# AI4Science-WestlakeU/safediffcon

Measured on AMD Instinct MI355X. Metric: sampled control trajectories/sec (1000-step DDPM), higher is better.
Workload: dtype f32; 1 GPU; C4: 2D smoke Unet3D_with_Conv3D dim=64 (1,2,4) state (B,32,7,64,64), B=64 per GPU, guided 1000-step DDPM, conformal quantile on; batch_per_gpu=64, global_batch=64, step=U-Net + guidance + posterior update of the whole batch, one hipGraph replay, parallelism=batch-sharded x1, no data-path collective, conv_precision=fp32

## Files before the change

### safediffcon_amd/csrc/sdc_conv_stem_x3.hip

```cpp
#include "sdc_conv.h"

using namespace sdcconv;

namespace {

typedef __bf16 bf16x8 __attribute__((ext_vector_type(8)));

constexpr int SX_BM = 64, SX_BN = 256, SX_NT = 256;

struct StemX3Args {
    const float* x;
    const __bf16* wb;
    const float* bias;
    float* y;
    int64_t xs[5], ys[5];
    int B, Cin, Cout, oD, oH, W, lgW;
    int kD;
    int Hs, NR;
    int Ntot, ntiles, mtiles;
    int itemsB;
    int plane;
};

__device__ __forceinline__ void split3(float x, __bf16& h, __bf16& m, __bf16& l) {
#pragma clang fp contract(off)
    h = (__bf16)x;
    const float r = x - (float)h;
    m = (__bf16)r;
    l = (__bf16)(r - (float)m);
}

template <int KH, int ITB>
__global__ __launch_bounds__(SX_NT) __attribute__((amdgpu_waves_per_eu(1))) SDC_NO_DS_MERGE void conv_stem_x3_kernel(const StemX3Args a) {
    constexpr int TAPS = KH * 7;
    constexpr int NS = (TAPS + 1) / 2;
    constexpr int SS = KH == 7 ? 5 : NS;
    constexpr int NSUB = NS / SS;
    static_assert(NSUB * SS == NS, "whole sub-stages");
    constexpr int HH = KH - 1;
    constexpr int APC = SS * SX_BM * 32;
    constexpr int ASZ = 3 * APC;
    constexpr int NIA = 3 * SS * SX_BM * 2;
    constexpr int ITA = (NIA + SX_NT - 1) / SX_NT;
    extern __shared__ __attribute__((aligned(16))) char lds[];

    const int tid = threadIdx.x, lane = tid & 63, wave = tid >> 6;
    const int l31 = lane & 31, lh = lane >> 5;
    const int W = a.W, RP = W + 6;
    const int BIMG = a.NR * RP * 16;
    const int logical = xcd_tile(blockIdx.x, a.ntiles * a.mtiles);
    const int mt = logical % a.mtiles, nt = logical / a.mtiles;
    const int m0 = mt * SX_BM, n0 = nt * SX_BN;
    const int r0 = n0 >> a.lgW;
    const int plane0 = r0 / a.oH, oh0 = r0 - plane0 * a.oH;
    const int GR = a.Hs + HH;

    int64_t bb[ITB];
    int bod[ITB], bdst[ITB];
    bool bok[ITB];
#pragma unroll
    for (int k = 0; k < ITB; ++k) {
        const int it = tid + k * SX_NT;
        const int w = it & (W - 1);
        const int sr = it >> a.lgW;
        int pl, ih;
        if (KH == 1) { const int row = r0 + sr; pl = row / a.oH; ih = row - pl * a.oH; }
        else { const int g = sr / GR, q = sr - g * GR; pl = plane0 + g; ih = (g == 0 ? oh0 : 0) - 3 + q; }
        const bool ok = it < a.itemsB && pl < a.B * a.oD && ih >= 0 && ih < a.oH;
        const int b = ok ? pl / a.oD : 0, od = ok ? pl % a.oD : 0, ihc = ok ? ih : 0;
        bok[k] = ok;
        bod[k] = od;
        bb[k] = (int64_t)b * a.xs[0] + (int64_t)od * a.xs[2] + (int64_t)ihc * a.xs[3] + (int64_t)w;
        bdst[k] = ASZ + (sr * RP + w + 3) * 16;
    }
    int aoff[ITA];
#pragma unroll
    for (int k = 0; k < ITA; ++k) {
        const int it = tid + k * SX_NT;
        const int p = it / (SS * 2 * SX_BM), q = it - p * (SS * 2 * SX_BM);
        const int s = q / (2 * SX_BM), r = q - s * (2 * SX_BM);
        aoff[k] = it < NIA ? p * a.plane + (s * a.Cout + m0) * 16 + r * 8 : 0;
    }

    float bv[ITB][8];
    uint4 av[ITA];
    auto load_a = [&](int kd, int sub) {
        const int wst = (kd * NS + sub * SS) * a.Cout * 16;
#pragma unroll
        for (int k = 0; k < ITA; ++k) {
            uint4 v = make_uint4(0u, 0u, 0u, 0u);
            if (tid + k * SX_NT < NIA) v = *reinterpret_cast<const uint4*>(a.wb + wst + aoff[k]);
            av[k] = v;
        }
    };
    auto load_b = [&](int kd) {
        const int dk = kd - a.kD / 2;
#pragma unroll
        for (int k = 0; k < ITB; ++k) {
            const int sd = bod[k] + dk;
            const bool ok = bok[k] && sd >= 0 && sd < a.oD;
            const float* q = a.x + bb[k] + (int64_t)dk * a.xs[2];
#pragma unroll
            for (int i = 0; i < 8; ++i) { bv[k][i] = (ok && i < a.Cin) ? *q : 0.0f; q += a.xs[1]; }
        }
    };
    auto store_a = [&]() {
#pragma unroll
        for (int k = 0; k < ITA; ++k)
            if (tid + k * SX_NT < NIA) *reinterpret_cast<uint4*>(lds + (tid + k * SX_NT) * 16) = av[k];
    };
    auto store_b = [&]() {
#pragma unroll
        for (int k = 0; k < ITB; ++k) {
            if (tid + k * SX_NT < a.itemsB) {
                bf16x8 h, m, l;
#pragma unroll
                for (int i = 0; i < 8; ++i) { __bf16 ph, pm, pl; split3(bv[k][i], ph, pm, pl); h[i] = ph; m[i] = pm; l[i] = pl; }
                *reinterpret_cast<bf16x8*>(lds + bdst[k]) = h;
                *reinterpret_cast<bf16x8*>(lds + bdst[k] + BIMG) = m;
                *reinterpret_cast<bf16x8*>(lds + bdst[k] + 2 * BIMG) = l;
            }
        }
    };

    for (int e = tid; e < 3 * a.NR * 6; e += SX_NT) {
        const int sr = e / 6, c = e - sr * 6;
        *reinterpret_cast<uint4*>(lds + ASZ + (sr * RP + (c < 3 ? c : W + c)) * 16) = make_uint4(0u, 0u, 0u, 0u);
    }

    int bA[2], bB[2], bC[2];
    constexpr int LAST_OFF = 16 * 6;
#pragma unroll
    for (int j = 0; j < 2; ++j) {
        const int p = wave * 64 + 32 * j + l31;
        const bool pok = n0 + p < a.Ntot;
        const int rl = pok ? p >> a.lgW : 0, col = pok ? p & (W - 1) : 0;
        int slot;
        if (KH == 1) slot = rl;
        else {
            const int row = r0 + rl, pl = row / a.oH, oh = row - pl * a.oH, g = pl - plane0;
            slot = g * GR + oh - (g == 0 ? oh0 : 0);
        }
        const int base = ASZ + (slot * RP + col) * 16;
        bA[j] = base + 16 * lh;
        bB[j] = base + lh * (RP * 16 - 16 * 6);
        bC[j] = lh ? ASZ - (HH * RP * 16 + LAST_OFF) : base;
    }
    const int aoffr = l31 * 32 + 16 * lh;
    const int rowb = RP * 16;

    f32x16 acc[2][2], sm[2][2];
#pragma unroll
    for (int i = 0; i < 2; ++i)
#pragma unroll
        for (int j = 0; j < 2; ++j)
#pragma unroll
            for (int r = 0; r < 16; ++r) {
                acc[i][j][r] = 0.0f;
                sm[i][j][r] = 0.0f;
            }

    load_a(0, 0);
    load_b(0);
    for (int kd = 0; kd < a.kD; ++kd) {
#pragma unroll
        for (int sub = 0; sub < NSUB; ++sub) {
            __syncthreads();
            store_a();
            if (sub == 0) store_b();
            __syncthreads();
            if (sub + 1 < NSUB) load_a(kd, sub + 1);
            else if (kd + 1 < a.kD) { load_a(kd + 1, 0); load_b(kd + 1); }
#pragma unroll
            for (int sl = 0; sl < SS; ++sl) {
                const int s = sub * SS + sl;
                const int t0 = 2 * s, kh = t0 / 7, kw = t0 - 7 * kh;
                const int tb = kh * rowb + kw * 16;
                bf16x8 af[2][3], bf[2][3];
#pragma unroll
                for (int i = 0; i < 2; ++i)
#pragma unroll
                    for (int p = 0; p < 3; ++p)
                        af[i][p] = *reinterpret_cast<const bf16x8*>(lds + p * APC + (sl * SX_BM + 32 * i) * 32 + aoffr);
#pragma unroll
                for (int j = 0; j < 2; ++j) {
                    const int bs = (s == NS - 1) ? bC[j] : (kw == 6 ? bB[j] : bA[j]);
#pragma unroll
                    for (int p = 0; p < 3; ++p) bf[j][p] = *reinterpret_cast<const bf16x8*>(lds + bs + tb + p * BIMG);
                }
                constexpr int PA[6] = {2, 1, 0, 1, 0, 0}, PB[6] = {0, 1, 2, 0, 1, 0};
#pragma unroll
                for (int t = 0; t < 6; ++t)
#pragma unroll
                    for (int i = 0; i < 2; ++i)
#pragma unroll
                        for (int j = 0; j < 2; ++j) {
                            f32x16& c = t < 5 ? sm[i][j] : acc[i][j];
                            c = __builtin_amdgcn_mfma_f32_32x32x16_bf16(af[i][PA[t]], bf[j][PB[t]], c, 0, 0, 0);
                        }
            }
        }
    }

#pragma unroll
    for (int i = 0; i < 2; ++i)
#pragma unroll
        for (int j = 0; j < 2; ++j) acc[i][j] += sm[i][j];
    float bz[2][16];
#pragma unroll
    for (int i = 0; i < 2; ++i)
#pragma unroll
        for (int rr = 0; rr < 16; ++rr) bz[i][rr] = 0.0f;
    if (a.bias) {
#pragma unroll
        for (int i = 0; i < 2; ++i)
#pragma unroll
            for (int rr = 0; rr < 16; ++rr) bz[i][rr] = a.bias[m0 + 32 * i + 4 * lh + (rr & 3) + 8 * (rr >> 2)];
    }
#pragma unroll
    for (int j = 0; j < 2; ++j) {
        const int p = n0 + wave * 64 + 32 * j + l31;
        if (p >= a.Ntot) continue;
        const int row = p >> a.lgW, col = p & (W - 1);
        const int pl = row / a.oH, oh = row - pl * a.oH;
        const int b = pl / a.oD, od = pl - b * a.oD;
        float* yp = a.y + (int64_t)b * a.ys[0] + (int64_t)od * a.ys[2] + (int64_t)oh * a.ys[3] + (int64_t)col
                    + (int64_t)(m0 + 4 * lh) * a.ys[1];
#pragma unroll
        for (int i = 0; i < 2; ++i) {
#pragma unroll
            for (int rr = 0; rr < 16; ++rr)
                yp[(int64_t)(32 * i + (rr & 3) + 8 * (rr >> 2)) * a.ys[1]] = acc[i][j][rr] + bz[i][rr];
        }
    }
}

__global__ __launch_bounds__(256) void pack_stem_x3_kernel(const float* __restrict__ w, __bf16* __restrict__ out, int Cout, int Cin, int kD,
                                                           int taps, int NS, int64_t n) {
    const int64_t e = (int64_t)blockIdx.x * 256 + threadIdx.x;
    if (e >= n) return;
    const int ci = (int)(e & 7), h = (int)((e >> 3) & 1);
    int64_t r = e >> 4;
    const int co = (int)(r % Cout); r /= Cout;
    const int s = (int)(r % NS);
    const int kd = (int)(r / NS);
    const int t = 2 * s + h;
    const float v = (ci < Cin && t < taps) ? w[(((int64_t)co * Cin + ci) * kD + kd) * taps + t] : 0.0f;
    __bf16 ph, pm, pl;
    split3(v, ph, pm, pl);
    out[e] = ph; out[n + e] = pm; out[2 * n + e] = pl;
}

}

namespace sdcconv {

int launch_stem_x3(const SdcConvDesc& d, const float* x, const __bf16* wb, const float* bias, float* y, hipStream_t s) {
    SDC_REQUIRE(reinterpret_cast<uintptr_t>(wb) % 16 == 0, SDC_EALIGN, "sdc_conv_stem_x3: the packed weight buffer must be 16-byte aligned");
    const StemShape sh = stem_shape(d);
    const int NS = (d.kH * 7 + 1) / 2, SS = d.kH == 7 ? 5 : NS;
    const size_t lds = (size_t)3 * SS * SX_BM * 32 + (size_t)3 * sh.NR * (d.oW + 6) * 16;
    SDC_REQUIRE(sh.itemsB <= 8 * SX_NT && lds <= 160u * 1024u, SDC_EINVAL, "sdc_conv_stem_x3: staging of %d positions / %zu bytes of LDS",
                sh.itemsB, lds);
    StemX3Args a;
    a.x = x; a.wb = wb; a.bias = bias; a.y = y;
    for (int i = 0; i < 5; ++i) { a.xs[i] = d.x0s[i]; a.ys[i] = d.ys[i]; }
    a.B = d.B; a.Cin = d.Cin0; a.Cout = d.Cout; a.oD = d.oD; a.oH = d.oH; a.W = d.oW;
    a.lgW = d.oW == 16 ? 4 : d.oW == 32 ? 5 : d.oW == 64 ? 6 : 7;
    a.kD = d.kD;
    a.Hs = sh.Hs; a.NR = sh.NR;
    const int64_t ntot = (int64_t)d.B * d.oD * d.oH * d.oW;
    SDC_REQUIRE(ntot < (1ll << 31), SDC_EINVAL, "sdc_conv_stem_x3: too many output positions");
    const int64_t plane = (int64_t)d.kD * NS * d.Cout * 16;
    SDC_REQUIRE(3 * plane < (1ll << 31), SDC_EINVAL, "sdc_conv_stem_x3: weight too large");
    a.plane = (int)plane;
    a.Ntot = (int)ntot;
    a.ntiles = (a.Ntot + SX_BN - 1) / SX_BN; a.mtiles = d.Cout / SX_BM;
    a.itemsB = sh.itemsB;
    SDC_REQUIRE((int64_t)a.ntiles * a.mtiles < (1ll << 31), SDC_EINVAL, "sdc_conv_stem_x3: grid too large");
    const dim3 grid((unsigned)(a.ntiles * a.mtiles));
#define STEM_LAUNCH(KH, ITB)                                                                                        \
    do {                                                                                                            \
        static std::atomic<uint64_t> attr{0};                                                                       \
        SDC_LDS_OPTIN(attr, (conv_stem_x3_kernel<KH, ITB>), 160 * 1024, "sdc_conv_stem_x3");                        \
        hipLaunchKernelGGL((conv_stem_x3_kernel<KH, ITB>), grid, dim3(SX_NT), lds, s, a);                           \
    } while (0)
    if (d.kH == 1) STEM_LAUNCH(1, 1);
    else if (sh.itemsB <= 2 * SX_NT) STEM_LAUNCH(7, 2);
    else if (sh.itemsB <= 4 * SX_NT) STEM_LAUNCH(7, 4);
    else STEM_LAUNCH(7, 8);
#undef STEM_LAUNCH
    return sdc::check_launch("sdc_conv_stem_x3");
}

}

extern "C" size_t sdc_pack_stem_x3_bytes(int Cout, int Cin, int kD, int kH, int kW) {
    return 3 * sdc_pack_stem_f16_bytes(Cout, Cin, kD, kH, kW);
}

extern "C" int sdc_pack_stem_x3(const float* w, void* out, int Cout, int Cin, int kD, int kH, int kW, void* stream) {
    SDC_REQUIRE(w && out, SDC_ENULL, "sdc_pack_stem_x3: null pointer");
    SDC_REQUIRE(sdc_pack_stem_x3_bytes(Cout, Cin, kD, kH, kW) > 0, SDC_EINVAL,
                "sdc_pack_stem_x3: taps 1x1x7, 1x7x7 or 7x7x7 and 1 <= Cin <= 8 (got %dx%dx%d, Cin %d, Cout %d)", kD, kH, kW, Cin, Cout);
    const int NS = (kH * 7 + 1) / 2;
    const int64_t n = (int64_t)kD * NS * Cout * 16;
    SDC_REQUIRE(n / 256 + 1 < (1ll << 31), SDC_EINVAL, "sdc_pack_stem_x3: weight too large");
    hipLaunchKernelGGL(pack_stem_x3_kernel, dim3((unsigned)((n + 255) / 256)), dim3(256), 0, sdc::as_stream(stream), w,
                       reinterpret_cast<__bf16*>(out), Cout, Cin, kD, kH * 7, NS, n);
    return sdc::check_launch("sdc_pack_stem_x3");
}
```

Measured before the change: 0.2930 trajectories/s.

## Double-buffer weight staging and software-pipeline fragment reads in bf16x3 stem conv

Adds a PIPE variant of the 7x7 bf16x3 stem convolution. It double-buffers the weight tile in LDS and prefetches the next sub-stage's fragments into registers while the current MFMAs run. Scheduling barriers interleave LDS reads with MFMAs, and the number of block-wide syncs per sub-stage drops. This targets exposed LDS and global latency in a single-wave-per-EU kernel, at the cost of more LDS and more registers for the doubled fragments. It also adds debug knobs gated behind an experiments macro.

```diff
diff --git a/safediffcon_amd/csrc/sdc_conv_stem_x3.hip b/safediffcon_amd/csrc/sdc_conv_stem_x3.hip
--- a/safediffcon_amd/csrc/sdc_conv_stem_x3.hip
+++ b/safediffcon_amd/csrc/sdc_conv_stem_x3.hip
@@ -20,6 +20,12 @@
     int Ntot, ntiles, mtiles;
     int itemsB;
     int plane;
+#ifdef SDC_KERNEL_EXPERIMENTS
+    int dbg;
+#define SX_DBG(a) ((a).dbg)
+#else
+#define SX_DBG(a) 0
+#endif
 };
 
 __device__ __forceinline__ void split3(float x, __bf16& h, __bf16& m, __bf16& l) {
@@ -30,7 +36,7 @@
     l = (__bf16)(r - (float)m);
 }
 
-template <int KH, int ITB>
+template <int KH, int ITB, bool PIPE>
 __global__ __launch_bounds__(SX_NT) __attribute__((amdgpu_waves_per_eu(1))) SDC_NO_DS_MERGE void conv_stem_x3_kernel(const StemX3Args a) {
     constexpr int TAPS = KH * 7;
     constexpr int NS = (TAPS + 1) / 2;
@@ -42,6 +48,7 @@
     constexpr int ASZ = 3 * APC;
     constexpr int NIA = 3 * SS * SX_BM * 2;
     constexpr int ITA = (NIA + SX_NT - 1) / SX_NT;
+    constexpr int BOFF = PIPE ? 2 * ASZ : ASZ;
     extern __shared__ __attribute__((aligned(16))) char lds[];
 
     const int tid = threadIdx.x, lane = tid & 63, wave = tid >> 6;
@@ -71,7 +78,7 @@
         bok[k] = ok;
         bod[k] = od;
         bb[k] = (int64_t)b * a.xs[0] + (int64_t)od * a.xs[2] + (int64_t)ihc * a.xs[3] + (int64_t)w;
-        bdst[k] = ASZ + (sr * RP + w + 3) * 16;
+        bdst[k] = BOFF + (sr * RP + w + 3) * 16;
     }
     int aoff[ITA];
 #pragma unroll
@@ -89,7 +96,7 @@
 #pragma unroll
         for (int k = 0; k < ITA; ++k) {
             uint4 v = make_uint4(0u, 0u, 0u, 0u);
-            if (tid + k * SX_NT < NIA) v = *reinterpret_cast<const uint4*>(a.wb + wst + aoff[k]);
+            if (tid + k * SX_NT < NIA && !(SX_DBG(a) & 4)) v = *reinterpret_cast<const uint4*>(a.wb + wst + aoff[k]);
             av[k] = v;
         }
     };
@@ -98,16 +105,16 @@
 #pragma unroll
         for (int k = 0; k < ITB; ++k) {
             const int sd = bod[k] + dk;
-            const bool ok = bok[k] && sd >= 0 && sd < a.oD;
+            const bool ok = bok[k] && sd >= 0 && sd < a.oD && !(SX_DBG(a) & 4);
             const float* q = a.x + bb[k] + (int64_t)dk * a.xs[2];
 #pragma unroll
             for (int i = 0; i < 8; ++i) { bv[k][i] = (ok && i < a.Cin) ? *q : 0.0f; q += a.xs[1]; }
         }
     };
-    auto store_a = [&]() {
+    auto store_a = [&](int abuf) {
 #pragma unroll
         for (int k = 0; k < ITA; ++k)
-            if (tid + k * SX_NT < NIA) *reinterpret_cast<uint4*>(lds + (tid + k * SX_NT) * 16) = av[k];
+            if (tid + k * SX_NT < NIA) *reinterpret_cast<uint4*>(lds + abuf + (tid + k * SX_NT) * 16) = av[k];
     };
     auto store_b = [&]() {
 #pragma unroll
@@ -125,7 +132,7 @@
 
     for (int e = tid; e < 3 * a.NR * 6; e += SX_NT) {
         const int sr = e / 6, c = e - sr * 6;
-        *reinterpret_cast<uint4*>(lds + ASZ + (sr * RP + (c < 3 ? c : W + c)) * 16) = make_uint4(0u, 0u, 0u, 0u);
+        *reinterpret_cast<uint4*>(lds + BOFF + (sr * RP + (c < 3 ? c : W + c)) * 16) = make_uint4(0u, 0u, 0u, 0u);
     }
 
     int bA[2], bB[2], bC[2];
@@ -141,10 +148,10 @@
             const int row = r0 + rl, pl = row / a.oH, oh = row - pl * a.oH, g = pl - plane0;
             slot = g * GR + oh - (g == 0 ? oh0 : 0);
         }
-        const int base = ASZ + (slot * RP + col) * 16;
+        const int base = BOFF + (slot * RP + col) * 16;
         bA[j] = base + 16 * lh;
         bB[j] = base + lh * (RP * 16 - 16 * 6);
-        bC[j] = lh ? ASZ - (HH * RP * 16 + LAST_OFF) : base;
+        bC[j] = lh ? BOFF - (HH * RP * 16 + LAST_OFF) : base;
     }
     const int aoffr = l31 * 32 + 16 * lh;
     const int rowb = RP * 16;
@@ -160,45 +167,114 @@
                 sm[i][j][r] = 0.0f;
             }
 
-    load_a(0, 0);
-    load_b(0);
-    for (int kd = 0; kd < a.kD; ++kd) {
-#pragma unroll
-        for (int sub = 0; sub < NSUB; ++sub) {
-            __syncthreads();
-            store_a();
-            if (sub == 0) store_b();
-            __syncthreads();
-            if (sub + 1 < NSUB) load_a(kd, sub + 1);
-            else if (kd + 1 < a.kD) { load_a(kd + 1, 0); load_b(kd + 1); }
-#pragma unroll
-            for (int sl = 0; sl < SS; ++sl) {
-                const int s = sub * SS + sl;
-                const int t0 = 2 * s, kh = t0 / 7, kw = t0 - 7 * kh;
-                const int tb = kh * rowb + kw * 16;
-                bf16x8 af[2][3], bf[2][3];
-#pragma unroll
-                for (int i = 0; i < 2; ++i)
-#pragma unroll
-                    for (int p = 0; p < 3; ++p)
-                        af[i][p] = *reinterpret_cast<const bf16x8*>(lds + p * APC + (sl * SX_BM + 32 * i) * 32 + aoffr);
+    auto read_frags = [&](bf16x8 (&af)[2][3], bf16x8 (&bf)[2][3], int abuf, int sl, int s) {
+        const int t0 = 2 * s, kh = t0 / 7, kw = t0 - 7 * kh;
+        const int tb = kh * rowb + kw * 16;
+#pragma unroll
+        for (int i = 0; i < 2; ++i)
+#pragma unroll
+            for (int p = 0; p < 3; ++p)
+                af[i][p] = *reinterpret_cast<const bf16x8*>(lds + abuf + p * APC + (sl * SX_BM + 32 * i) * 32 + aoffr);
+#pragma unroll
+        for (int j = 0; j < 2; ++j) {
+            const int bs = (s == NS - 1) ? bC[j] : (kw == 6 ? bB[j] : bA[j]);
+#pragma unroll
+            for (int p = 0; p < 3; ++p) bf[j][p] = *reinterpret_cast<const bf16x8*>(lds + bs + tb + p * BIMG);
+        }
+    };
+    auto mfmas = [&](const bf16x8 (&af)[2][3], const bf16x8 (&bf)[2][3]) {
+        constexpr int PA[6] = {2, 1, 0, 1, 0, 0}, PB[6] = {0, 1, 2, 0, 1, 0};
+#pragma unroll
+        for (int t = 0; t < 6; ++t)
+#pragma unroll
+            for (int i = 0; i < 2; ++i)
 #pragma unroll
                 for (int j = 0; j < 2; ++j) {
-                    const int bs = (s == NS - 1) ? bC[j] : (kw == 6 ? bB[j] : bA[j]);
-#pragma unroll
-                    for (int p = 0; p < 3; ++p) bf[j][p] = *reinterpret_cast<const bf16x8*>(lds + bs + tb + p * BIMG);
+                    f32x16& c = t < 5 ? sm[i][j] : acc[i][j];
+                    c = __builtin_amdgcn_mfma_f32_32x32x16_bf16(af[i][PA[t]], bf[j][PB[t]], c, 0, 0, 0);
                 }
-                constexpr int PA[6] = {2, 1, 0, 1, 0, 0}, PB[6] = {0, 1, 2, 0, 1, 0};
-#pragma unroll
-                for (int t = 0; t < 6; ++t)
-#pragma unroll
-                    for (int i = 0; i < 2; ++i)
-#pragma unroll
-                        for (int j = 0; j < 2; ++j) {
-                            f32x16& c = t < 5 ? sm[i][j] : acc[i][j];
-                            c = __builtin_amdgcn_mfma_f32_32x32x16_bf16(af[i][PA[t]], bf[j][PB[t]], c, 0, 0, 0);
+    };
+
+    auto interleave = [&]() {
+#pragma unroll
+        for (int r = 0; r < 12; ++r) {
+            __builtin_amdgcn_sched_group_barrier(0x100, 1, 0);
+            __builtin_amdgcn_sched_group_barrier(0x008, 2, 0);
+        }
+    };
+
+    if constexpr (PIPE) {
+        load_a(0, 0);
+        load_b(0);
+        store_a(0);
+        store_b();
+        if (1 / NSUB < a.kD) load_a(1 / NSUB, 1 % NSUB);
+        __syncthreads();
+        int abuf = 0;
+        for (int kd = 0; kd < a.kD; ++kd) {
+            bf16x8 fa[2][2][3], fb[2][2][3];
+            read_frags(fa[0], fb[0], abuf, 0, 0);
+#pragma unroll
+            for (int sub = 0; sub < NSUB; ++sub) {
+                if (kd + (sub + 1) / NSUB < a.kD) store_a(abuf ^ ASZ);
+                if (kd + (sub + 2) / NSUB < a.kD) load_a(kd + (sub + 2) / NSUB, (sub + 2) % NSUB);
+                if (sub == NSUB - 1 && kd + 1 < a.kD) load_b(kd + 1);
+#pragma unroll
+                for (int sl = 0; sl < SS; ++sl) {
+                    const int s = sub * SS + sl, cur = s & 1;
+                    if (sl + 1 < SS) {
+                        __builtin_amdgcn_sched_barrier(0);
+                        read_frags(fa[cur ^ 1], fb[cur ^ 1], abuf, sl + 1, s + 1);
+                        mfmas(fa[cur], fb[cur]);
+                        interleave();
+                        __builtin_amdgcn_sched_barrier(0);
+                    } else if (sub + 1 < NSUB) {
+                        __syncthreads();
+                        __builtin_amdgcn_sched_barrier(0);
+                        read_frags(fa[cur ^ 1], fb[cur ^ 1], abuf ^ ASZ, 0, s + 1);
+                        mfmas(fa[cur], fb[cur]);
+                        interleave();
+                        __builtin_amdgcn_sched_barrier(0);
+                    } else {
+                        const bool more = kd + 1 < a.kD;
+                        if (more) {
+                            __syncthreads();
+                            store_b();
                         }
+                        mfmas(fa[cur], fb[cur]);
+                        if (more) __syncthreads();
+                    }
+                }
+                abuf ^= ASZ;
             }
+        }
+    } else {
+        bf16x8 af[2][3], bf[2][3];
+        const int dbg = SX_DBG(a);
+        load_a(0, 0);
+        load_b(0);
+        if (dbg & 1) read_frags(af, bf, 0, 0, 0);
+        for (int kd = 0; kd < ((dbg & 8) ? 0 : a.kD); ++kd) {
+#pragma unroll
+            for (int sub = 0; sub < NSUB; ++sub) {
+                if (!(dbg & 2)) {
+                    __syncthreads();
+                    store_a(0);
+                    if (sub == 0) store_b();
+                    __syncthreads();
+                }
+                if (sub + 1 < NSUB) load_a(kd, sub + 1);
+                else if (kd + 1 < a.kD) { load_a(kd + 1, 0); load_b(kd + 1); }
+#pragma unroll
+                for (int sl = 0; sl < SS; ++sl) {
+                    if (!(dbg & 1)) read_frags(af, bf, 0, sl, sub * SS + sl);
+                    mfmas(af, bf);
+                }
+            }
+        }
+        if (dbg & 6) {
+            store_a(0);
+            store_b();
         }
     }
 
@@ -259,7 +335,12 @@
     SDC_REQUIRE(reinterpret_cast<uintptr_t>(wb) % 16 == 0, SDC_EALIGN, "sdc_conv_stem_x3: the packed weight buffer must be 16-byte aligned");
     const StemShape sh = stem_shape(d);
     const int NS = (d.kH * 7 + 1) / 2, SS = d.kH == 7 ? 5 : NS;
-    const size_t lds = (size_t)3 * SS * SX_BM * 32 + (size_t)3 * sh.NR * (d.oW + 6) * 16;
+    bool pipe = d.kH == 7 && sh.itemsB <= 4 * SX_NT;
+#ifdef SDC_KERNEL_EXPERIMENTS
+    static const int dbg = exp_env("SDC_X3_DBG");
+    if (dbg) pipe = false;
+#endif
+    const size_t lds = (size_t)(pipe ? 2 : 1) * 3 * SS * SX_BM * 32 + (size_t)3 * sh.NR * (d.oW + 6) * 16;
     SDC_REQUIRE(sh.itemsB <= 8 * SX_NT && lds <= 160u * 1024u, SDC_EINVAL, "sdc_conv_stem_x3: staging of %d positions / %zu bytes of LDS",
                 sh.itemsB, lds);
     StemX3Args a;
@@ -277,18 +358,27 @@
     a.Ntot = (int)ntot;
     a.ntiles = (a.Ntot + SX_BN - 1) / SX_BN; a.mtiles = d.Cout / SX_BM;
     a.itemsB = sh.itemsB;
+#ifdef SDC_KERNEL_EXPERIMENTS
+    a.dbg = dbg & 15;
+#endif
     SDC_REQUIRE((int64_t)a.ntiles * a.mtiles < (1ll << 31), SDC_EINVAL, "sdc_conv_stem_x3: grid too large");
     const dim3 grid((unsigned)(a.ntiles * a.mtiles));
-#define STEM_LAUNCH(KH, ITB)                                                                                        \
+#define STEM_LAUNCH(KH, ITB, PIPE)                                                                                  \
     do {                                                                                                            \
         static std::atomic<uint64_t> attr{0};                                                                       \
-        SDC_LDS_OPTIN(attr, (conv_stem_x3_kernel<KH, ITB>), 160 * 1024, "sdc_conv_stem_x3");                        \
-        hipLaunchKernelGGL((conv_stem_x3_kernel<KH, ITB>), grid, dim3(SX_NT), lds, s, a);                           \
+        SDC_LDS_OPTIN(attr, (conv_stem_x3_kernel<KH, ITB, PIPE>), 160 * 1024, "sdc_conv_stem_x3");                  \
+        hipLaunchKernelGGL((conv_stem_x3_kernel<KH, ITB, PIPE>), grid, dim3(SX_NT), lds, s, a);                     \
     } while (0)
-    if (d.kH == 1) STEM_LAUNCH(1, 1);
-    else if (sh.itemsB <= 2 * SX_NT) STEM_LAUNCH(7, 2);
-    else if (sh.itemsB <= 4 * SX_NT) STEM_LAUNCH(7, 4);
-    else STEM_LAUNCH(7, 8);
+#ifdef SDC_KERNEL_EXPERIMENTS
+    if (!pipe && d.kH == 7 && sh.itemsB <= 4 * SX_NT) {
+        if (sh.itemsB <= 2 * SX_NT) STEM_LAUNCH(7, 2, false);
+        else STEM_LAUNCH(7, 4, false);
+    } else
+#endif
+    if (d.kH == 1) STEM_LAUNCH(1, 1, false);
+    else if (sh.itemsB <= 2 * SX_NT) STEM_LAUNCH(7, 2, true);
+    else if (sh.itemsB <= 4 * SX_NT) STEM_LAUNCH(7, 4, true);
+    else STEM_LAUNCH(7, 8, false);
 #undef STEM_LAUNCH
     return sdc::check_launch("sdc_conv_stem_x3");
 }
```

New measurement: 0.2937 trajectories/s, median of 2. Within noise of the previous version (+0.3%).
